# MariusFurter/WeightedSampling.jl

Hardware: AMD Instinct MI355X
Metric: particle-steps/sec (N_particles × T_steps / wall-s), 2D SSM bootstrap filter (higher is better)
Workload: dtype f64; 1 GPU; 2D SSM bootstrap filter (examples/2D_ssm.jl), BASELINE configs[1]; n_particles_per_gpu=1000000, global_particles=1000000, T=100, scheme=stratified, keep_history=True, estimator=reference (single population), parallelism=single GPU

## Files before the change

include/wsmc_math.h:

```cpp
#ifndef WSMC_MATH_H
#define WSMC_MATH_H

#include <stdint.h>

#if defined(__HIPCC__) || defined(__HIP__)
#define WSMC_HD __host__ __device__ inline __attribute__((always_inline))
#else
#define WSMC_HD static inline __attribute__((always_inline))
#endif
#if defined(__clang__)
#define WSMC_UNROLL _Pragma("unroll")
#else
#define WSMC_UNROLL _Pragma("GCC unroll 16")
#endif

typedef unsigned __int128 wsmc_u128;

#if defined(__HIP_DEVICE_COMPILE__)
__device__ inline __attribute__((always_inline)) double wsmc_sreg(double c) {
    __asm__ volatile("" : "+s"(c));
    return c;
}
#define WSMC_K(c) wsmc_sreg(c)
#else
// ... 557 lines not shown
        const double t = y * wsmc_lgamma_g(y);
        return n >= 3.0 ? wsmc_log(z) + t : t;
    }
    const double r = 1.0 / x;
    const double z = r * r;
    double q = WSMC_K(-0.020855820837463117);
    q = __builtin_fma(q, z, WSMC_K(0.0062081367662297935));
    q = __builtin_fma(q, z, WSMC_K(-0.001914965912162907));
    q = __builtin_fma(q, z, WSMC_K(0.0008417325268022405));
    q = __builtin_fma(q, z, WSMC_K(-0.0005952380234291254));
    q = __builtin_fma(q, z, WSMC_K(0.0007936507935117282));
    q = __builtin_fma(q, z, WSMC_K(-0.0027777777777776747));
    q = __builtin_fma(q, z, WSMC_K(0.08333333333333333));
    const double w = __builtin_fma(q, r, 0.4189385332046727);
    const double lx = wsmc_log(x);
    if (lx == WSMC_INF) return lx;
    return __builtin_fma(x - 0.5, lx - 1.0, w);
}
WSMC_HD double wsmc_lgamma3(double a1, double a2, double a3) {
    double acc = 0.0;
#if defined(__clang__)
#pragma nounroll
#endif
    for (int k = 0; k < 3; ++k) {
        const double a = k == 0 ? a1 : (k == 1 ? a2 : a3);
        const double l = a == 1.0 ? 0.0 : wsmc_lgamma(a);
        acc = k == 0 ? l : acc - l;
    }
    return acc;
}
WSMC_HD double wsmc_lbeta(double a, double b) { return -wsmc_lgamma3(a + b, a, b); }
WSMC_HD double wsmc_lchoose(double n, double k) { return wsmc_lgamma3(n + 1.0, k + 1.0, (n - k) + 1.0); }

WSMC_HD void wsmc_normal_pair_t(wsmc_u32x4 w, double* z0, double* z1, const double* logtab) {
    double u1 = wsmc_u01_open0(w.v[0], w.v[1]);
    double u2 = wsmc_u01(w.v[2], w.v[3]);
    double r = wsmc_sqrt(-2.0 * wsmc_log_t(u1, logtab));
    double s, c;
    wsmc_sincos2pi(u2, &s, &c);
    *z0 = r * c; *z1 = r * s;
}
WSMC_HD void wsmc_normal_pair(wsmc_u32x4 w, double* z0, double* z1) { wsmc_normal_pair_t(w, z0, z1, WSMC_LOG_TAB); }
WSMC_HD double wsmc_normal_k(uint64_t seed, uint64_t op, uint64_t idx, uint32_t k) {
    double z0, z1;
    wsmc_normal_pair(wsmc_rng_block(seed, op, idx, k >> 1), &z0, &z1);
    return (k & 1) ? z1 : z0;
}
WSMC_HD double wsmc_uniform_k(uint64_t seed, uint64_t op, uint64_t idx, uint32_t k) {
    wsmc_u32x4 w = wsmc_rng_block(seed, op, idx, (k >> 1) | 0x80u);
    return (k & 1) ? wsmc_u01(w.v[2], w.v[3]) : wsmc_u01(w.v[0], w.v[1]);
}
WSMC_HD uint64_t wsmc_strat_key(uint64_t seed, uint64_t op) {
    uint64_t z = seed ^ (op * 0x9E3779B97F4A7C15ULL) ^ 0x5851F42D4C957F2DULL;
    z ^= z >> 33;
    z *= 0xFF51AFD7ED558CCDULL;
    z ^= z >> 33;
    z *= 0xC4CEB9FE1A85EC53ULL;
    z ^= z >> 33;
    return z;
}
WSMC_HD uint32_t wsmc_strat_fin(uint32_t x) {
    x ^= x >> 16;
    x *= 0x7FEB352Du;
    x ^= x >> 15;
    x *= 0x846CA68Bu;
    x ^= x >> 16;
    return x;
}
WSMC_HD uint32_t wsmc_strat_hash(uint64_t key, uint64_t n) {
    return wsmc_strat_fin((uint32_t)n ^ (uint32_t)key ^ ((uint32_t)(n >> 32) * 0x85EBCA6Bu ^ (uint32_t)(key >> 32)));
}
WSMC_HD uint32_t wsmc_strat_word(uint64_t seed, uint64_t op, uint64_t n) {
    return wsmc_strat_hash(wsmc_strat_key(seed, op), n);
// ... 355 lines not shown
```

weightedsampling.jl_amd/build.py:

```python
from __future__ import annotations

import argparse
import os
import pathlib
import shutil
import subprocess
import sys
from concurrent.futures import ThreadPoolExecutor

PKG = pathlib.Path(__file__).resolve().parent
REPO = PKG.parent
CSRC = PKG / "csrc"
INCLUDE = REPO / "include"
OUT = PKG / "wsmc" / "libwsmc.so"
OBJDIR = PKG / "build"
RESOURCES = OBJDIR / "wsmc_kernels.resources.txt"
SOURCES = ["wsmc_kernels.hip", "wsmc_api.hip", "wsmc_multi.hip", "wsmc_jit.hip", "wsmc_lgssm.hip"]
JIT_HEADERS = [INCLUDE / "wsmc.h", INCLUDE / "wsmc_log_table.h", INCLUDE / "wsmc_exp_table.h", INCLUDE / "wsmc_math.h", INCLUDE / "wsmc_terms.h", CSRC / "wsmc_ew.h",
               CSRC / "wsmc_ew_body.h", CSRC / "wsmc_mv.h", CSRC / "wsmc_mv_body.h"]
ARCH = os.environ.get("WSMC_OFFLOAD_ARCH", "gfx950")


def hipcc() -> str:
    for cand in (os.environ.get("HIPCC"), "/opt/rocm/bin/hipcc", shutil.which("hipcc")):
        if cand and pathlib.Path(cand).exists():
            return cand
    raise RuntimeError("hipcc not found")


COMMON = ["-O3", "-std=c++17", "-fPIC", "-ffp-contract=off", "-fno-fast-math",
          f"--offload-arch={ARCH}", "-I", str(INCLUDE), "-I", str(CSRC),
          "-Wno-unused-result", "-munsafe-fp-atomics"]


def _deps():
    return [CSRC / s for s in SOURCES] + list(CSRC.glob("*.h")) + list(INCLUDE.glob("*.h"))


def up_to_date() -> bool:
    if not OUT.exists() or not RESOURCES.exists():
        return False
    t = OUT.stat().st_mtime
    return all(p.stat().st_mtime <= t for p in _deps())


def write_jit_headers() -> pathlib.Path:
    out = OBJDIR / "wsmc_jit_headers.inc"
    parts = []
    for h in JIT_HEADERS:
        text = h.read_text()
        assert ")WSMCJIT\"" not in text
        parts.append(f'{{"{h.name}", R"WSMCJIT({text})WSMCJIT"}},')
    body = "// generated by build.py: the headers of the run-time compiled kernels\n" + "\n".join(parts) + "\n"
    if not out.exists() or out.read_text() != body:
        out.write_text(body)
    return out


def build(force: bool = False, verbose: bool = False) -> pathlib.Path:
    if not force and up_to_date():
        return OUT
    OBJDIR.mkdir(exist_ok=True)
    write_jit_headers()
    cc = hipcc()

    def compile_one(src: str) -> pathlib.Path:
        obj = OBJDIR / (pathlib.Path(src).stem + ".o")
        cmd = [cc, *COMMON, "-I", str(OBJDIR), "-c", str(CSRC / src), "-o", str(obj)]
        listing = src == "wsmc_kernels.hip"
        if listing:
            cmd.append("-Rpass-analysis=kernel-resource-usage")
        if verbose:
            print(" ".join(cmd), flush=True)
        r = subprocess.run(cmd, capture_output=True, text=True)
        if r.returncode != 0:
            raise RuntimeError(f"hipcc failed on {src}:\n{r.stdout}\n{r.stderr}")
        if listing:
            tail = " [-Rpass-analysis=kernel-resource-usage]"
            remarks = [ln.split("remark: ", 1)[1].replace(tail, "") for ln in r.stderr.splitlines() if "remark: " in ln]
            RESOURCES.write_text("\n".join(remarks) + "\n")
        if verbose and r.stderr and not listing:
            print(r.stderr, file=sys.stderr)
        return obj

    with ThreadPoolExecutor(max_workers=len(SOURCES)) as ex:
        objs = list(ex.map(compile_one, SOURCES))
    tmp = OUT.with_suffix(".so.tmp")
    cmd = [cc, f"--offload-arch={ARCH}", "-shared", "-fPIC", *map(str, objs), "-o", str(tmp),
           "-L/opt/rocm/lib", "-lrccl", "-lhiprtc", "-Wl,-rpath,/opt/rocm/lib"]
    if verbose:
        print(" ".join(cmd), flush=True)
    r = subprocess.run(cmd, capture_output=True, text=True)
    if r.returncode != 0:
        raise RuntimeError(f"link failed:\n{r.stdout}\n{r.stderr}")
    os.replace(tmp, OUT)
    return OUT


if __name__ == "__main__":
    ap = argparse.ArgumentParser()
    ap.add_argument("--force", action="store_true")
    ap.add_argument("--verbose", action="store_true")
    a = ap.parse_args()
    print(build(force=a.force, verbose=a.verbose))
```

weightedsampling.jl_amd/csrc/wsmc_api.hip:

```cpp
#include <hipcub/hipcub.hpp>

#include <algorithm>
#include <chrono>
#include <memory>
#include <thread>
#include <cmath>
#include <cstdio>
#include <cstring>
#include <string>

#include "wsmc_internal.h"

using namespace wsmc;

namespace wsmc {
bool peer_aborted(wsmc_ctx* c) {
    if (!c->peer_abort || !c->peer_abort->load(std::memory_order_acquire)) return false;
    if (c->comm) {
        (void)ncclCommAbort(c->comm);
        c->comm = nullptr;
    }
    c->released = true;
    return true;
}
// ... 555 lines not shown
int wsmc_dist_mvnormal_cov(wsmc_dist* d, const double* cov) {
    if (!d || !cov) return fail(WSMC_EARG, "null argument");
    if (d->dim < 1 || d->dim > WSMC_MVN_MAXDIM) return fail(WSMC_EARG, "MvNormal with a full covariance: dim must be 1..3");
    if (d->mean_fn != WSMC_MEAN_AFFINE) return fail(WSMC_EARG, "MvNormal mean must be affine");
    const int r = wsmc_mvn_pack(d, cov);
    if (r == -1) return fail(WSMC_EARG, "covariance is not symmetric");
    if (r == -2) return fail(WSMC_ENOTPD, "covariance is not positive definite");
    return WSMC_OK;
}

int wsmc_device_count(int32_t* n) {
    int k = 0;
    WSMC_HIP(hipGetDeviceCount(&k));
    *n = k;
    return WSMC_OK;
}

int wsmc_create(wsmc_ctx** out, int64_t n_particles, int32_t device, uint64_t seed) {
    if (!out) return fail(WSMC_EARG, "null out");
    if (n_particles < 1 || n_particles >= (int64_t(1) << 31))
        return fail(WSMC_EARG, "n_particles must be in [1, 2^31)");
    WSMC_HIP(hipSetDevice(device));
    wsmc_ctx* c = new wsmc_ctx();
    c->device = device;
    c->N = n_particles;
    c->gN = n_particles;
    c->seed = seed;
    c->ntiles = (n_particles + kTile - 1) / kTile;
    c->nrstiles = (n_particles + kRsTile - 1) / kRsTile;
    hipError_t e = hipSuccess;
#define ALLOC(ptr, bytes)                                          \
    if (e == hipSuccess) e = hipMalloc((void**)&(ptr), (bytes));
    e = hipStreamCreateWithFlags(&c->stream, hipStreamNonBlocking);
    ALLOC(c->w, sizeof(double) * c->N);
    ALLOC(c->anc, sizeof(int32_t) * c->N);
    ALLOC(c->tmp, sizeof(double) * 4 * c->N);
    ALLOC(c->xchg, sizeof(unsigned long long) * 16 * kMaxWorld);
    ALLOC(c->tilep, sizeof(unsigned long long) * kPart * c->nrstiles);
    ALLOC(c->tileOff, sizeof(unsigned long long) * c->nrstiles);
    ALLOC(c->taskOff, sizeof(int32_t) * c->nrstiles);
    ALLOC(c->taskTile, sizeof(int32_t) * (c->nrstiles + n_particles / kRsChunk + 1));
    ALLOC(c->mslots, sizeof(MaxSlots));
    ALLOC(c->wslots[0], sizeof(MaxSlots));
    ALLOC(c->wslots[1], sizeof(MaxSlots));
    ALLOC(c->qbuf, sizeof(unsigned long long) * c->N);
    ALLOC(c->tilepart, sizeof(double) * 64 * c->ntiles);
    ALLOC(c->rec, sizeof(ShardRecord) * kMaxWorld);
    ALLOC(c->dec, sizeof(Decision));
    ALLOC(c->dec_always, sizeof(Decision));
    ALLOC(c->mom, sizeof(double) * 128);
    ALLOC(c->dflag, sizeof(int32_t) * 4);
    ALLOC(c->ucount, sizeof(unsigned long long) * (4 * kAccMove + 4));
    ALLOC(c->d_colptr, sizeof(double*) * kMaxCols);
    ALLOC(c->run_params, sizeof(uint64_t) * 8);
#undef ALLOC
    if (e == hipSuccess) e = hipHostMalloc(&c->pinned, 4096, hipHostMallocDefault);
    if (e == hipSuccess) e = hipHostMalloc((void**)&c->dec_ring, sizeof(Decision) * kDecRing, hipHostMallocDefault);
    if (e == hipSuccess) e = hipHostGetDevicePointer((void**)&c->dec_ring_dev, c->dec_ring, 0);
    if (e == hipSuccess) e = hipHostGetDevicePointer(&c->pinned_dev, c->pinned, 0);
    if (e == hipSuccess) e = hipMemsetAsync(c->w, 0, sizeof(double) * c->N, c->stream);
    if (e == hipSuccess) e = hipMemsetAsync(c->wslots[0], 0, sizeof(MaxSlots), c->stream);
    if (e == hipSuccess) e = hipMemsetAsync(c->wslots[1], 0, sizeof(MaxSlots), c->stream);
    if (e == hipSuccess) e = hipMemsetAsync(c->anc, 0, sizeof(int32_t) * c->N, c->stream);
    if (e == hipSuccess) {
        Decision always{};
        always.resampled = 1;
        e = hipMemcpy(c->dec_always, &always, sizeof(Decision), hipMemcpyHostToDevice);
    }
    if (e == hipSuccess) e = ctx_sync(c, c->stream);
    {
        const char* eg = getenv("WSMC_EAGER_GATHER");
        c->lazy = !(eg && atoi(eg) != 0);
    }
    if (e != hipSuccess) {
        std::string m = std::string("wsmc_create: ") + hipGetErrorString(e);
        wsmc_destroy(c);
        return fail(WSMC_EHIP, m);
    }
// ... 4203 lines not shown
```

weightedsampling.jl_amd/csrc/wsmc_kernels.hip:

```cpp
#include <hip/hip_ext.h>

#include <cstdlib>
#include "wsmc_internal.h"

namespace wsmc {

typedef double d2 __attribute__((ext_vector_type(2)));

typedef unsigned long long u64;

#ifdef WSMC_DIAG_BUILD
constexpr int kClkKinds = 4, kClkBlocks = 16384;
__device__ u64 g_blk_clk[kClkKinds][kClkBlocks][2];
struct BlkClock {
    int kind;
    u64 t0;
    __device__ __forceinline__ explicit BlkClock(int k) : kind(k), t0(wall_clock64()) {}
    __device__ __forceinline__ ~BlkClock() {
        if (threadIdx.x == 0 && blockIdx.x < (unsigned)kClkBlocks) {
            g_blk_clk[kind][blockIdx.x][0] = t0;
            g_blk_clk[kind][blockIdx.x][1] = wall_clock64();
        }
    }
};
// ... 20 lines not shown
}
__device__ __forceinline__ u64 lane63_u64(u64 v) {
    const uint32_t lo = (uint32_t)__builtin_amdgcn_readlane((int)(uint32_t)v, 63);
    const uint32_t hi = (uint32_t)__builtin_amdgcn_readlane((int)(uint32_t)(v >> 32), 63);
    return ((u64)hi << 32) | lo;
}
__device__ __forceinline__ u64 wave_sum_u64(u64 v) {
    v += dpp_u64<kDppQuad1032>(v);
    v += dpp_u64<kDppQuad2301>(v);
    v += dpp_u64<kDppRowRor4>(v);
    v += dpp_u64<kDppRowRor8>(v);
    v += dpp_u64<kDppBcast15>(v);
    v += dpp_u64<kDppBcast31>(v);
    return lane63_u64(v);
}
__device__ __forceinline__ u64 wave_max_u64(u64 v) {
    u64 o;
    o = dpp_u64<kDppQuad1032>(v); v = o > v ? o : v;
    o = dpp_u64<kDppQuad2301>(v); v = o > v ? o : v;
    o = dpp_u64<kDppRowRor4>(v); v = o > v ? o : v;
    o = dpp_u64<kDppRowRor8>(v); v = o > v ? o : v;
    o = dpp_u64<kDppBcast15>(v); v = o > v ? o : v;
    o = dpp_u64<kDppBcast31>(v); v = o > v ? o : v;
    return lane63_u64(v);
}
__device__ __forceinline__ double wave_sum_f64_exact(double v) {
    v = v + dpp_f64<kDppQuad1032>(v);
    v = v + dpp_f64<kDppQuad2301>(v);
    v = v + dpp_f64<kDppRowRor4>(v);
    v = v + dpp_f64<kDppRowRor8>(v);
    v = v + dpp_f64<kDppBcast15>(v);
    v = v + dpp_f64<kDppBcast31>(v);
    return __builtin_bit_cast(double, lane63_u64(__builtin_bit_cast(u64, v)));
}
__device__ __forceinline__ u64 wave_incl_scan_u64(u64 v) {
    u64 x = v + dpp_u64<kDppRowShr1>(v);
    x += dpp_u64<kDppRowShr2>(v);
    x += dpp_u64<kDppRowShr3>(v);
    x += dpp_u64<kDppRowShr4, 0xf, 0xe>(x);
    x += dpp_u64<kDppRowShr8, 0xf, 0xc>(x);
    x += dpp_u64<kDppBcast15, 0xa, 0xf>(x);
    x += dpp_u64<kDppBcast31, 0xc, 0xf>(x);
    return x;
}
__device__ __forceinline__ double block_sum_canon(double v, double* lds4) {
#pragma unroll
    for (int off = 1; off < 64; off <<= 1) v = v + __shfl_xor(v, off, 64);
    if ((threadIdx.x & 63) == 0) lds4[threadIdx.x >> 6] = v;
    __syncthreads();
    double r = (lds4[0] + lds4[1]) + (lds4[2] + lds4[3]);
    __syncthreads();
    return r;
}
__device__ __forceinline__ u64 block_sum_u64(u64 v, u64* lds4) {
    v = wave_sum_u64(v);
    if ((threadIdx.x & 63) == 0) lds4[threadIdx.x >> 6] = v;
    __syncthreads();
    u64 r = (lds4[0] + lds4[1]) + (lds4[2] + lds4[3]);
    __syncthreads();
    return r;
}
__device__ __forceinline__ u64 block_max_u64(u64 v, u64* lds4) {
    v = wave_max_u64(v);
    if ((threadIdx.x & 63) == 0) lds4[threadIdx.x >> 6] = v;
    __syncthreads();
    u64 a = lds4[0] > lds4[1] ? lds4[0] : lds4[1];
// ... 879 lines not shown
            if (dd < -kMargin) return ns;
        }
    }
    return wsmc_rank_r(c, Q, N, ratio, scheme, seed, op, slot_base);
}

template <int CTRL, int ROW = 0xf, int BANK = 0xf>
__device__ __forceinline__ int dpp_i32_or(int v, int idn) {
    return __builtin_amdgcn_update_dpp(idn, v, CTRL, ROW, BANK, false);
}
__device__ __forceinline__ int wave_incl_max_i32(int v) {
    int x = max(v, dpp_i32_or<kDppRowShr1>(v, -1));
    x = max(x, dpp_i32_or<kDppRowShr2>(v, -1));
    x = max(x, dpp_i32_or<kDppRowShr3>(v, -1));
    x = max(x, dpp_i32_or<kDppRowShr4, 0xf, 0xe>(x, -1));
    x = max(x, dpp_i32_or<kDppRowShr8, 0xf, 0xc>(x, -1));
    x = max(x, dpp_i32_or<kDppBcast15, 0xa, 0xf>(x, -1));
    x = max(x, dpp_i32_or<kDppBcast31, 0xc, 0xf>(x, -1));
    return x;
}
__device__ __forceinline__ double wave_incl_scan_f64(double v) {
    double x = v + dpp_f64<kDppRowShr1>(v);
    x = x + dpp_f64<kDppRowShr2>(v);
    x = x + dpp_f64<kDppRowShr3>(v);
    x = x + __builtin_bit_cast(double, dpp_u64<kDppRowShr4, 0xf, 0xe>(__builtin_bit_cast(u64, x)));
    x = x + __builtin_bit_cast(double, dpp_u64<kDppRowShr8, 0xf, 0xc>(__builtin_bit_cast(u64, x)));
    x = x + __builtin_bit_cast(double, dpp_u64<kDppBcast15, 0xa, 0xf>(__builtin_bit_cast(u64, x)));
    x = x + __builtin_bit_cast(double, dpp_u64<kDppBcast31, 0xc, 0xf>(__builtin_bit_cast(u64, x)));
    return x;
}

template <int IT>
__device__ __forceinline__ void load_tile_q(int64_t N, int b, const u64* __restrict__ qbuf, u64 (&q)[IT]) {
#pragma unroll
    for (int k = 0; k < IT; ++k) {
        const int64_t i = (int64_t)b * kRsTile + (int64_t)threadIdx.x * IT + k;
        q[k] = i < N ? qbuf[i] : 0ull;
    }
}

template <int IT>
__device__ __forceinline__ void load_tile_qw(int64_t N, int b, const double* __restrict__ w,
                                             const MaxSlots* __restrict__ ms, const double* rref, u64 (&q)[IT]) {
    double lw[IT];
#pragma unroll
    for (int k = 0; k < IT; ++k) {
        const int64_t i = (int64_t)b * kRsTile + (int64_t)threadIdx.x * IT + k;
        lw[k] = i < N ? w[i] : -WSMC_INF;
    }
    const double R = rref ? *rref : wsmc_qref(wave_slots_max(ms));
    const double sK = wsmc_pow2i(wsmc_qbits((uint64_t)N));
#pragma unroll
    for (int k = 0; k < IT; ++k) {
        double e = wsmc_expw(lw[k] - R);
        e = e > 0.0 ? e : 0.0;
        q[k] = d_small_to_u64(wsmc_floor(e * sK));
    }
}

__device__ __forceinline__ void fill_clear(FillLds& sh) {
    const int4 m1 = make_int4(-1, -1, -1, -1);
    int4* o = reinterpret_cast<int4*>(sh.out);
    o[2 * threadIdx.x] = m1;
    o[2 * threadIdx.x + 1] = m1;
    if (threadIdx.x == 0) o[2 * kScanBlock] = m1;
}

__device__ __forceinline__ void fill_store4(int32_t* __restrict__ dst, int p0, int a, int e, int4 v) {
    if (p0 >= a && p0 + 4 <= e) {
        *reinterpret_cast<int4*>(dst + p0) = v;
    } else if (p0 + 4 > a && p0 < e) {
        if (p0 >= a && p0 < e) dst[p0] = v.x;
        if (p0 + 1 >= a && p0 + 1 < e) dst[p0 + 1] = v.y;
        if (p0 + 2 >= a && p0 + 2 < e) dst[p0 + 2] = v.z;
        if (p0 + 3 >= a && p0 + 3 < e) dst[p0 + 3] = v.w;
    }
}

template <int MODE>
__device__ __forceinline__ void fill_chunk_core(int64_t N, int b, int j, u64 Q, u64 off, u64 qb, double pre,
                                                const FillPlan& plan, uint64_t opx,
                                                const u64 (&q)[kRsTile / kScanBlock], int32_t* __restrict__ anc,
// ... 583 lines not shown
        if ((th & 63) == 0)
#pragma unroll
            for (int k = 0; k < kRedPart; ++k) s_parts[th >> 6][k] = acc[k];
        __syncthreads();
        if (th == 0) {
            u64 tot[kRedPart] = {0, 0, 0, 0, 0, 0};
            for (int v = 0; v < kScanBlock / 64; ++v)
                for (int k = 0; k < kRedPart; ++k) tot[k] += s_parts[v][k];
            ShardRecord r;
            r.menc = menc;
            r.Q = tot[0];
            r.q2 = tot[1];
            const wsmc_u128 Wf2 = (wsmc_u128)tot[2] + ((wsmc_u128)tot[3] << 32);
            const wsmc_u128 Wf = (wsmc_u128)tot[4] + ((wsmc_u128)tot[5] << 32);
            r.wf2lo = (u64)Wf2; r.wf2hi = (u64)(Wf2 >> 64);
            r.wflo = (u64)Wf; r.wfhi = (u64)(Wf >> 64);
            r.n = (u64)N;
            *rec = r;
            if (plan.rg_check && !(wsmc_qref(wsmc_ord_dec(menc)) == *plan.rg_check)) atomicAdd(plan.rg_miss, 1);
            if (dec) {
                decide_records(&r, 1, 0, ess_min, dec);
                if (plan.host_dec) *plan.host_dec = *dec;
                if (plan.base_out) *plan.base_out = dec->resampled ? dec->mean : wsmc_ord_dec(menc);
                if (plan.ms_reset && dec->resampled) {
                    plan.ms_reset->v[0][0] = wsmc_ord_enc(dec->mean);
                    for (int k = 1; k < kSlots; ++k) plan.ms_reset->v[k][0] = 0ull;
                }
            }
        }
        return;
    }
    const uint64_t opx = op_eff(plan.op, plan.op_dev);
    if (t < ntiles) {
        u64 q[kRsTile / kScanBlock];
        if (QW)
            load_tile_qw(N, t, wq, ms, plan.rg_check, q);
        else
            load_tile_q(N, t, qbuf, q);
        const u64 qb = plan.tilep[(int64_t)t * kPart];
        const int g = t / G;
        u64 pre = 0, tot = 0;
        if (plan.xlines) {
            const int ngw = (int)(plan.xstride / kGroupLine);
            for (int k = th; k < plan.dx_world * ngw; k += kScanBlock) {
                const int r = k / ngw, kk = k - r * ngw;
                const u64 v = plan.xlines[(int64_t)r * plan.xstride + (int64_t)kk * kGroupLine];
                tot += v;
                pre += (r < plan.dx_rank || (r == plan.dx_rank && kk < g)) ? v : 0ull;
            }
        } else {
            for (int k = th; k < ngroups; k += kScanBlock) {
                const u64 v = grp[(int64_t)k * 8];
                tot += v;
                pre += k < g ? v : 0ull;
            }
        }
        for (int b = g * G + th; b < t; b += kScanBlock) pre += plan.tilep[(int64_t)b * kPart];
        fill_clear(sh);
        const int lane = th & 63, wv = th >> 6;
        pre = wave_sum_u64(pre);
        tot = wave_sum_u64(tot);
        const double tsum = tile_q_sum(q);
        const double x = wave_incl_scan_f64(tsum);
        if (lane == 63) {
            sh.uw[wv] = x;
            sh.red[wv][0] = pre;
            sh.red[wv][1] = tot;
        }
        __syncthreads();
        u64 off = 0, Q = 0;
        double lp = 0.0;
#pragma unroll
        for (int k = 0; k < kScanBlock / 64; ++k) {
            off += sh.red[k][0];
            Q += sh.red[k][1];
            if (k < wv) lp = lp + sh.uw[k];
        }
        fill_chunk_core<0>(N, t, 0, Q, off, qb, lp + (x - tsum), plan, opx, q, anc, sh, false);
        return;
    }
    u64 Q = 0, qmax = 0, cbase = 0;
    for (int k = th; k < ngroups; k += kScanBlock) {
        Q += grp[(int64_t)k * kGroupLine];
        const u64 m = grp[(int64_t)k * kGroupLine + 1];
        qmax = m > qmax ? m : qmax;
    }
    if (plan.xlines) {
        Q = 0;
        const int ngw = (int)(plan.xstride / kGroupLine);
        for (int k = th; k < plan.dx_world * ngw; k += kScanBlock) {
            const int r = k / ngw, kk = k - r * ngw;
            const u64 v = plan.xlines[(int64_t)r * plan.xstride + (int64_t)kk * kGroupLine];
            Q += v;
            cbase += r < plan.dx_rank ? v : 0ull;
        }
    }
    qmax = block_max_u64(qmax, s_u);
    block_sum2_u64(Q, cbase, s_red);
    const uint64_t Nr = plan.n_global ? plan.n_global : (uint64_t)N;
    const double ratio = Q ? wsmc_u64_to_d(Nr) / wsmc_u64_to_d(Q) : 0.0;
    if (ovf_chunks(qmax, ratio) == 0) return;

    const int per = (ntiles + kScanBlock - 1) / kScanBlock;
    const int b0 = th * per < ntiles ? th * per : ntiles;
    const int b1 = b0 + per < ntiles ? b0 + per : ntiles;
    u64 qs = 0, ns = 0;
    for (int b = b0; b < b1; ++b) {
        const u64 qb = plan.tilep[(int64_t)b * kPart];
        qs += qb;
        ns += (u64)ovf_chunks(qb, ratio);
    }
    u64 qtot, ntasks;
    const u64 qpre = block_excl_scan_u64<kScanBlock / 64>(qs, s_u, &qtot);
    const u64 npre = block_excl_scan_u64<kScanBlock / 64>(ns, s_u, &ntasks);
    __shared__ uint32_t s_npre[kScanBlock], s_ns[kScanBlock];
    __shared__ u64 s_c0[kScanBlock];
    s_npre[th] = (uint32_t)npre;
    s_ns[th] = (uint32_t)ns;
    s_c0[th] = cbase + qpre;
    const u64 Qu = ((u64)__builtin_amdgcn_readfirstlane((int)(Q >> 32)) << 32) |
                   (uint32_t)__builtin_amdgcn_readfirstlane((int)(uint32_t)Q);
    const uint32_t nt = (uint32_t)__builtin_amdgcn_readfirstlane((int)(uint32_t)ntasks);
    for (uint32_t o = (uint32_t)(t - ntiles); o < nt; o += kOverflowBlocks) {
        const uint32_t n0_ = s_npre[th], k_ = s_ns[th];
        if (o >= n0_ && o < n0_ + k_) {
            u64 c = s_c0[th];
            uint32_t n0 = n0_;
            const int per_ = (ntiles + kScanBlock - 1) / kScanBlock;
            const int bb0 = th * per_ < ntiles ? th * per_ : ntiles;
            const int bb1 = bb0 + per_ < ntiles ? bb0 + per_ : ntiles;
            for (int b = bb0; b < bb1; ++b) {
                const u64 qb = plan.tilep[(int64_t)b * kPart];
                const uint32_t k = (uint32_t)ovf_chunks(qb, ratio);
                if (o < n0 + k) {
// ... 1037 lines not shown
    const bool isl = QS ? ISL : (a.recs_prev != nullptr && a.t > 1);
    const bool identity = !QS && a.identity;
    const int64_t stride = (int64_t)gridDim.x * NT * 2;
    const int64_t ib = ((int64_t)blockIdx.x * NT + threadIdx.x) * 2;
    int2 s2[IT];
    bool ok[IT], two[IT];
#pragma unroll
    for (int j = 0; j < IT; ++j) {
        const int64_t i0 = ib + (int64_t)j * stride;
        ok[j] = i0 < N;
        two[j] = i0 + 1 < N;
        s2[j] = int2{0, 0};
        if (QS && (MODE & 2) == 0) {
            s2[j] = *reinterpret_cast<const int2*>(a.anc_prev + (ok[j] ? i0 : 0));
        } else if (ok[j] && !first && (MODE & 2) == 0 && !identity) {
            if (two[j]) {
                s2[j] = *reinterpret_cast<const int2*>(a.anc_prev + i0);
            } else {
                s2[j].x = a.anc_prev[i0];
            }
        }
    }
    u64 mprev = 0;
    if (QS) mprev = a.ms_prev->v[threadIdx.x & 63][0];
    if (isl) {
        if (threadIdx.x == 0) {
            Decision dd;
            decide_records(a.recs_prev, a.world, a.rank, a.ess_min, &dd);
            s_dec = dd;
            if (blockIdx.x == 0) *a.dec_out = dd;
        }
    }
    const uint64_t op_dv = a.op_dev[0] + 3ull * (uint64_t)(a.t - 1);
    const double o0 = a.obs[2 * (a.t - 1)], o1 = a.obs[2 * (a.t - 1) + 1];
    bool rs = false;
    double mean = 0.0;
    if (!isl && !first) {
        rs = a.dec_prev->resampled;
        mean = rs ? a.dec_prev->mean : 0.0;
    }
    if (WSMC_PROP_LDS_LOG && (MODE & 1) == 0) {
        const double* lt = wsmc_log_table();
        for (int k = (int)threadIdx.x; k < 2 * WSMC_LOG_TABLE_N; k += NT) s_logtab[k] = lt[k];
    }
    if ((WSMC_PROP_LDS_LOG && (MODE & 1) == 0) || isl) __syncthreads();
    const double* logtab = WSMC_PROP_LDS_LOG ? s_logtab : wsmc_log_table();
    if (isl) {
        rs = s_dec.resampled;
        mean = rs ? s_dec.mean : 0.0;
    }
    int64_t src[IT][2];
#pragma unroll
    for (int j = 0; j < IT; ++j) {
        const int64_t i0 = ib + (int64_t)j * stride;
        src[j][0] = i0; src[j][1] = i0 + 1;
        if (ok[j] && !first && (MODE & 2) == 0 && !identity && rs) { src[j][0] = s2[j].x; src[j][1] = s2[j].y; }
    }
    d2 xp[IT][2], vp[IT][2];
    double wb[IT][2];
#pragma unroll
    for (int j = 0; j < IT; ++j) {
        const int64_t i0 = ib + (int64_t)j * stride;
        wb[j][0] = wb[j][1] = mean;
        if (!ok[j]) continue;
        if (!rs) {
            if (two[j]) {
                const d2 w2 = *reinterpret_cast<const d2*>(a.w + i0);
                wb[j][0] = w2.x; wb[j][1] = w2.y;
                if (!QS && a.w_save) *reinterpret_cast<d2*>(a.w_save + i0) = w2;
            } else {
                wb[j][0] = a.w[i0];
                if (!QS && a.w_save) a.w_save[i0] = wb[j][0];
            }
        }
#pragma unroll
        for (int k = 0; k < 2; ++k) {
            if (first) {
                xp[j][k] = d2{a.x0[0], a.x0[1]};
                vp[j][k] = d2{a.v0[0], a.v0[1]};
            } else if (k == 0 || two[j]) {
                if (MODE & 16) {
                    const int64_t loc = rs ? src[j][k] - a.goff : src[j][k];
                    const bool here = loc >= 0 && loc < N;
                    const double* xs = here ? a.x_prev + 2 * loc : a.xr + 2 * (i0 + k);
                    const double* vs = here ? a.v_prev + 2 * loc : a.vr + 2 * (i0 + k);
                    xp[j][k] = *reinterpret_cast<const d2*>(xs);
                    vp[j][k] = *reinterpret_cast<const d2*>(vs);
                } else {
                    xp[j][k] = *reinterpret_cast<const d2*>(a.x_prev + 2 * src[j][k]);
                    vp[j][k] = *reinterpret_cast<const d2*>(a.v_prev + 2 * src[j][k]);
                }
            }
        }
    }
    u64 menc = 0;
    QAcc acc;
    double Rg = 0.0, sK = 0.0;
    if (QS) {
        const double base = rs ? mean : wsmc_ord_dec(wave_max_u64(mprev));
        const double lpmax = -(a.c0 + 0.0) * 0.5;
        Rg = wsmc_qref(base + lpmax);
        sK = wsmc_pow2i(wsmc_qbits((uint64_t)N));
        if (blockIdx.x == 0 && threadIdx.x == 0) *a.rg_out = Rg;
    }
#pragma unroll
    for (int j = 0; j < IT; ++j) {
        if (!ok[j]) continue;
        const int64_t i0 = ib + (int64_t)j * stride;
        double z[2][2] = {{0.0, 0.0}, {0.0, 0.0}};
        if ((MODE & 1) == 0) {
#pragma unroll
            for (int k = 0; k < 2; ++k)
                wsmc_normal_pair_t(wsmc_rng_block(a.seed, op_dv, (uint64_t)(a.goff + i0 + k), 0u), &z[k][0], &z[k][1],
                                   logtab);
        }
        d2 xn[2], vn[2], dvv[2];
        double wn[2];
#pragma unroll
        for (int k = 0; k < 2; ++k) {
            const double xn0 = aff2(xp[j][k].x, vp[j][k].x), xn1 = aff2(xp[j][k].y, vp[j][k].y);
            const double dv0 = 0.0 + a.q_sd * z[k][0], dv1 = 0.0 + a.q_sd * z[k][1];
            const double vn0 = aff2(vp[j][k].x, dv0), vn1 = aff2(vp[j][k].y, dv1);
            const double m0 = 0.0 + 1.0 * xn0, m1 = 0.0 + 1.0 * xn1;
            double s = 0.0;
            const double d0 = o0 - m0, d1 = o1 - m1;
            s = s + d0 * d0;
            s = s + d1 * d1;
            const double lp = -(a.c0 + s / a.r_var) * 0.5;
            wn[k] = wb[j][k] + lp;
            xn[k] = d2{xn0, xn1};
            vn[k] = d2{vn0, vn1};
            dvv[k] = d2{dv0, dv1};
        }
        *reinterpret_cast<d2*>(a.x_next + 2 * i0) = xn[0];
        *reinterpret_cast<d2*>(a.v_next + 2 * i0) = vn[0];
        if (a.dv) *reinterpret_cast<d2*>(a.dv + 2 * i0) = dvv[0];
        u64 e0 = wsmc_ord_enc(wn[0]);
        menc = e0 > menc ? e0 : menc;
        u64 q0 = 0, q1 = 0;
        if (QS) q0 = qacc_add(acc, wsmc_expw(wn[0] - Rg), sK);
        if (two[j]) {
            *reinterpret_cast<d2*>(a.x_next + 2 * i0 + 2) = xn[1];
            *reinterpret_cast<d2*>(a.v_next + 2 * i0 + 2) = vn[1];
            if (a.dv) *reinterpret_cast<d2*>(a.dv + 2 * i0 + 2) = dvv[1];
            *reinterpret_cast<d2*>(a.w + i0) = d2{wn[0], wn[1]};
            const u64 e1 = wsmc_ord_enc(wn[1]);
            menc = e1 > menc ? e1 : menc;
            if (QS) q1 = qacc_add(acc, wsmc_expw(wn[1] - Rg), sK);
            if (QS && a.qbuf) *reinterpret_cast<ulonglong2*>(a.qbuf + i0) = make_ulonglong2(q0, q1);
        } else {
            a.w[i0] = wn[0];
            if (QS && a.qbuf) a.qbuf[i0] = q0;
        }
    }
    if (QS) {
        __shared__ double s_f[kPart][NT / 64];
        const int th = threadIdx.x, wv = th >> 6;
        acc.Q = wave_sum_f64_exact(acc.Q);
        acc.Q2 = wave_sum_f64_exact(acc.Q2);
        acc.WF2 = wave_sum_f64_exact(acc.WF2);
        acc.WF = wave_sum_f64_exact(acc.WF);
        menc = wave_max_u64(menc);
        if ((th & 63) == 0) {
            s_f[0][wv] = acc.Q; s_f[1][wv] = acc.Q2;
            s_f[2][wv] = acc.WF2; s_f[3][wv] = acc.WF;
            lds4[wv] = menc;
        }
        __syncthreads();
        if (th < kPart) {
            double f = 0.0;
#pragma unroll
            for (int v = 0; v < NT / 64; ++v) f = f + s_f[th][v];
            const u64 t = (u64)f;
            a.tilep[(int64_t)blockIdx.x * kPart + th] = t;
            if (th == 0) {
                u64* gl = a.grp + (int64_t)(blockIdx.x / a.G) * kGroupLine;
                atomicAdd(gl, t);
                atomicMax(gl + 1, t);
            }
        } else if (th == 64) {
            u64 m = 0;
#pragma unroll
            for (int v = 0; v < NT / 64; ++v) m = lds4[v] > m ? lds4[v] : m;
            atomic_max_filtered(&a.ms->v[blockIdx.x % kSlots][0], m);
        }
        return;
    }
    if (MODE & 4) {
        if (menc == 0x123456789ull) a.w[0] = 0.0;
        return;
    }
    if (MODE & 8) {
        menc = wave_max_u64(menc);
        if ((threadIdx.x & 63) == 0) atomicMax(&a.ms->v[(blockIdx.x * 4 + (threadIdx.x >> 6)) % kSlots][0], menc);
        return;
    }
    menc = block_max_u64(menc, lds4);
    if (threadIdx.x == 0) atomic_max_filtered(&a.ms->v[blockIdx.x % kSlots][0], menc);
}

__global__ __launch_bounds__(kBlock) void k_trace_pack(const double* __restrict__ xpairs,
                                                       const int32_t* __restrict__ arow, int64_t start, int64_t count,
                                                       u64* __restrict__ out) {
    const int64_t j = (int64_t)blockIdx.x * kBlock + threadIdx.x;
    if (j >= count) return;
    const d2 x = *reinterpret_cast<const d2*>(xpairs + 2 * (start + j));
    out[3 * j] = (u64)wsmc_d2bits(x.x);
    out[3 * j + 1] = (u64)wsmc_d2bits(x.y);
    out[3 * j + 2] = arow ? (u64)(uint32_t)arow[start + j] : 0ull;
}
__global__ __launch_bounds__(kBlock) void k_trace_lookup(const u64* __restrict__ recv, int64_t lo,
                                                         const int32_t* __restrict__ a, int64_t n,
                                                         double* __restrict__ xout, int32_t* __restrict__ anext,
                                                         int use_a) {
    const int64_t i = (int64_t)blockIdx.x * kBlock + threadIdx.x;
    if (i >= n) return;
    const int64_t o = (int64_t)a[i] - lo;
    xout[i] = wsmc_bits2d(recv[3 * o]);
    xout[n + i] = wsmc_bits2d(recv[3 * o + 1]);
    anext[i] = use_a ? (int32_t)(uint32_t)recv[3 * o + 2] : a[i];
}
__global__ __launch_bounds__(kBlock) void k_pairs_to_soa(const double* __restrict__ pairs, double* __restrict__ soa,
                                                         int64_t n) {
    const int64_t i = (int64_t)blockIdx.x * kBlock + threadIdx.x;
    if (i >= n) return;
    const d2 v = *reinterpret_cast<const d2*>(pairs + 2 * i);
    soa[i] = v.x;
    soa[n + i] = v.y;
}
__global__ __launch_bounds__(kBlock) void k_fill_const2(double* __restrict__ soa, double v0, double v1, int64_t n) {
    const int64_t i = (int64_t)blockIdx.x * kBlock + threadIdx.x;
    if (i >= n) return;
// ... 1057 lines not shown
```

Baseline: 32.57 billion particle-steps/s.

## Split normal draws around log-table staging and vectorize tile/quad reductions

In the fused 2D SSM propagate kernel, the Box-Muller draw is split into a head (uniforms and sincos), computed before the LDS log-table barrier, and a tail (log and sqrt), so the RNG work overlaps the table staging. Kernel arguments are re-read late through an opaque kernarg pointer to lower scalar register pressure. The per-wave four-value reduction is merged into one permlane-swap tree. Loads in the resample scan are vectorized to quads, and its prefix loads are hoisted, which needs the weight and qbuf buffers padded to a multiple of four. The build also emits an ISA listing.

```diff
diff --git a/include/wsmc_math.h b/include/wsmc_math.h
--- a/include/wsmc_math.h
+++ b/include/wsmc_math.h
@@ -613,13 +613,18 @@
 WSMC_HD double wsmc_lbeta(double a, double b) { return -wsmc_lgamma3(a + b, a, b); }
 WSMC_HD double wsmc_lchoose(double n, double k) { return wsmc_lgamma3(n + 1.0, k + 1.0, (n - k) + 1.0); }
 
+WSMC_HD void wsmc_normal_pair_head(wsmc_u32x4 w, double* u1, double* s, double* c) {
+    *u1 = wsmc_u01_open0(w.v[0], w.v[1]);
+    wsmc_sincos2pi(wsmc_u01(w.v[2], w.v[3]), s, c);
+}
+WSMC_HD void wsmc_normal_pair_tail(double u1, double s, double c, double* z0, double* z1, const double* logtab) {
+    double r = wsmc_sqrt(-2.0 * wsmc_log_t(u1, logtab));
+    *z0 = r * c; *z1 = r * s;
+}
 WSMC_HD void wsmc_normal_pair_t(wsmc_u32x4 w, double* z0, double* z1, const double* logtab) {
-    double u1 = wsmc_u01_open0(w.v[0], w.v[1]);
-    double u2 = wsmc_u01(w.v[2], w.v[3]);
-    double r = wsmc_sqrt(-2.0 * wsmc_log_t(u1, logtab));
-    double s, c;
-    wsmc_sincos2pi(u2, &s, &c);
-    *z0 = r * c; *z1 = r * s;
+    double u1, s, c;
+    wsmc_normal_pair_head(w, &u1, &s, &c);
+    wsmc_normal_pair_tail(u1, s, c, z0, z1, logtab);
 }
 WSMC_HD void wsmc_normal_pair(wsmc_u32x4 w, double* z0, double* z1) { wsmc_normal_pair_t(w, z0, z1, WSMC_LOG_TAB); }
 WSMC_HD double wsmc_normal_k(uint64_t seed, uint64_t op, uint64_t idx, uint32_t k) {
diff --git a/weightedsampling.jl_amd/build.py b/weightedsampling.jl_amd/build.py
--- a/weightedsampling.jl_amd/build.py
+++ b/weightedsampling.jl_amd/build.py
@@ -15,6 +15,7 @@
 OUT = PKG / "wsmc" / "libwsmc.so"
 OBJDIR = PKG / "build"
 RESOURCES = OBJDIR / "wsmc_kernels.resources.txt"
+ISA = OBJDIR / "wsmc_kernels.s"
 SOURCES = ["wsmc_kernels.hip", "wsmc_api.hip", "wsmc_multi.hip", "wsmc_jit.hip", "wsmc_lgssm.hip"]
 JIT_HEADERS = [INCLUDE / "wsmc.h", INCLUDE / "wsmc_log_table.h", INCLUDE / "wsmc_exp_table.h", INCLUDE / "wsmc_math.h", INCLUDE / "wsmc_terms.h", CSRC / "wsmc_ew.h",
                CSRC / "wsmc_ew_body.h", CSRC / "wsmc_mv.h", CSRC / "wsmc_mv_body.h"]
@@ -38,7 +39,7 @@
 
 
 def up_to_date() -> bool:
-    if not OUT.exists() or not RESOURCES.exists():
+    if not OUT.exists() or not RESOURCES.exists() or not ISA.exists():
         return False
     t = OUT.stat().st_mtime
     return all(p.stat().st_mtime <= t for p in _deps())
@@ -83,8 +84,20 @@
             print(r.stderr, file=sys.stderr)
         return obj
 
-    with ThreadPoolExecutor(max_workers=len(SOURCES)) as ex:
+    def listing_isa() -> None:
+        tmp = ISA.with_suffix(".s.tmp")
+        cmd = [cc, *COMMON, "-I", str(OBJDIR), "--offload-device-only", "-S", str(CSRC / "wsmc_kernels.hip"), "-o", str(tmp)]
+        if verbose:
+            print(" ".join(cmd), flush=True)
+        r = subprocess.run(cmd, capture_output=True, text=True)
+        if r.returncode != 0:
+            raise RuntimeError(f"hipcc -S failed on wsmc_kernels.hip:\n{r.stdout}\n{r.stderr}")
+        os.replace(tmp, ISA)
+
+    with ThreadPoolExecutor(max_workers=len(SOURCES) + 1) as ex:
+        isa = ex.submit(listing_isa)
         objs = list(ex.map(compile_one, SOURCES))
+        isa.result()
     tmp = OUT.with_suffix(".so.tmp")
     cmd = [cc, f"--offload-arch={ARCH}", "-shared", "-fPIC", *map(str, objs), "-o", str(tmp),
            "-L/opt/rocm/lib", "-lrccl", "-lhiprtc", "-Wl,-rpath,/opt/rocm/lib"]
diff --git a/weightedsampling.jl_amd/csrc/wsmc_api.hip b/weightedsampling.jl_amd/csrc/wsmc_api.hip
--- a/weightedsampling.jl_amd/csrc/wsmc_api.hip
+++ b/weightedsampling.jl_amd/csrc/wsmc_api.hip
@@ -611,7 +611,7 @@
 #define ALLOC(ptr, bytes)                                          \
     if (e == hipSuccess) e = hipMalloc((void**)&(ptr), (bytes));
     e = hipStreamCreateWithFlags(&c->stream, hipStreamNonBlocking);
-    ALLOC(c->w, sizeof(double) * c->N);
+    ALLOC(c->w, sizeof(double) * ((c->N + 3) & ~(int64_t)3));
     ALLOC(c->anc, sizeof(int32_t) * c->N);
     ALLOC(c->tmp, sizeof(double) * 4 * c->N);
     ALLOC(c->xchg, sizeof(unsigned long long) * 16 * kMaxWorld);
@@ -622,7 +622,7 @@
     ALLOC(c->mslots, sizeof(MaxSlots));
     ALLOC(c->wslots[0], sizeof(MaxSlots));
     ALLOC(c->wslots[1], sizeof(MaxSlots));
-    ALLOC(c->qbuf, sizeof(unsigned long long) * c->N);
+    ALLOC(c->qbuf, sizeof(unsigned long long) * ((c->N + 3) & ~(int64_t)3));
     ALLOC(c->tilepart, sizeof(double) * 64 * c->ntiles);
     ALLOC(c->rec, sizeof(ShardRecord) * kMaxWorld);
     ALLOC(c->dec, sizeof(Decision));
diff --git a/weightedsampling.jl_amd/csrc/wsmc_kernels.hip b/weightedsampling.jl_amd/csrc/wsmc_kernels.hip
--- a/weightedsampling.jl_amd/csrc/wsmc_kernels.hip
+++ b/weightedsampling.jl_amd/csrc/wsmc_kernels.hip
@@ -76,6 +76,32 @@
     v = v + dpp_f64<kDppBcast15>(v);
     v = v + dpp_f64<kDppBcast31>(v);
     return __builtin_bit_cast(double, lane63_u64(__builtin_bit_cast(u64, v)));
+}
+__device__ __forceinline__ void lane_swap32(double& a, double& b) {
+    const u64 x = __builtin_bit_cast(u64, a), y = __builtin_bit_cast(u64, b);
+    const auto lo = __builtin_amdgcn_permlane32_swap((uint32_t)x, (uint32_t)y, false, false);
+    const auto hi = __builtin_amdgcn_permlane32_swap((uint32_t)(x >> 32), (uint32_t)(y >> 32), false, false);
+    a = __builtin_bit_cast(double, ((u64)hi[0] << 32) | lo[0]);
+    b = __builtin_bit_cast(double, ((u64)hi[1] << 32) | lo[1]);
+}
+__device__ __forceinline__ void lane_swap16(double& a, double& b) {
+    const u64 x = __builtin_bit_cast(u64, a), y = __builtin_bit_cast(u64, b);
+    const auto lo = __builtin_amdgcn_permlane16_swap((uint32_t)x, (uint32_t)y, false, false);
+    const auto hi = __builtin_amdgcn_permlane16_swap((uint32_t)(x >> 32), (uint32_t)(y >> 32), false, false);
+    a = __builtin_bit_cast(double, ((u64)hi[0] << 32) | lo[0]);
+    b = __builtin_bit_cast(double, ((u64)hi[1] << 32) | lo[1]);
+}
+__device__ __forceinline__ double wave_sum4_f64_exact(double v0, double v1, double v2, double v3) {
+    lane_swap32(v0, v2);
+    lane_swap32(v1, v3);
+    double a = v0 + v2, b = v1 + v3;
+    lane_swap16(a, b);
+    double r = a + b;
+    r = r + dpp_f64<kDppQuad1032>(r);
+    r = r + dpp_f64<kDppQuad2301>(r);
+    r = r + dpp_f64<kDppRowRor4>(r);
+    r = r + dpp_f64<kDppRowRor8>(r);
+    return r;
 }
 __device__ __forceinline__ u64 wave_incl_scan_u64(u64 v) {
     u64 x = v + dpp_u64<kDppRowShr1>(v);
@@ -1021,22 +1047,28 @@
 
 template <int IT>
 __device__ __forceinline__ void load_tile_q(int64_t N, int b, const u64* __restrict__ qbuf, u64 (&q)[IT]) {
-#pragma unroll
-    for (int k = 0; k < IT; ++k) {
-        const int64_t i = (int64_t)b * kRsTile + (int64_t)threadIdx.x * IT + k;
-        q[k] = i < N ? qbuf[i] : 0ull;
-    }
+    static_assert(IT == 4, "one quad a thread");
+    const int64_t i = (int64_t)b * kRsTile + (int64_t)threadIdx.x * IT;
+    const ulonglong2* p = reinterpret_cast<const ulonglong2*>(qbuf + (i < N ? i : 0));
+    const ulonglong2 lo = p[0], hi = p[1];
+    q[0] = i < N ? lo.x : 0ull;
+    q[1] = i + 1 < N ? lo.y : 0ull;
+    q[2] = i + 2 < N ? hi.x : 0ull;
+    q[3] = i + 3 < N ? hi.y : 0ull;
 }
 
 template <int IT>
 __device__ __forceinline__ void load_tile_qw(int64_t N, int b, const double* __restrict__ w,
                                              const MaxSlots* __restrict__ ms, const double* rref, u64 (&q)[IT]) {
+    static_assert(IT == 4, "one quad a thread");
+    const int64_t i = (int64_t)b * kRsTile + (int64_t)threadIdx.x * IT;
+    const d2* p = reinterpret_cast<const d2*>(w + (i < N ? i : 0));
+    const d2 lo = p[0], hi = p[1];
     double lw[IT];
-#pragma unroll
-    for (int k = 0; k < IT; ++k) {
-        const int64_t i = (int64_t)b * kRsTile + (int64_t)threadIdx.x * IT + k;
-        lw[k] = i < N ? w[i] : -WSMC_INF;
-    }
+    lw[0] = i < N ? lo.x : -WSMC_INF;
+    lw[1] = i + 1 < N ? lo.y : -WSMC_INF;
+    lw[2] = i + 2 < N ? hi.x : -WSMC_INF;
+    lw[3] = i + 3 < N ? hi.y : -WSMC_INF;
     const double R = rref ? *rref : wsmc_qref(wave_slots_max(ms));
     const double sK = wsmc_pow2i(wsmc_qbits((uint64_t)N));
 #pragma unroll
@@ -1686,13 +1718,16 @@
     }
     const uint64_t opx = op_eff(plan.op, plan.op_dev);
     if (t < ntiles) {
+        const u64 qb = plan.tilep[(int64_t)t * kPart];
+        const int g = t / G;
+        const u64 g0 = grp[(int64_t)(th < ngroups ? th : 0) * 8];
+        const int bf = g * G + th;
+        const u64 p0 = plan.tilep[(int64_t)(bf < t ? bf : t) * kPart];
         u64 q[kRsTile / kScanBlock];
         if (QW)
             load_tile_qw(N, t, wq, ms, plan.rg_check, q);
         else
             load_tile_q(N, t, qbuf, q);
-        const u64 qb = plan.tilep[(int64_t)t * kPart];
-        const int g = t / G;
         u64 pre = 0, tot = 0;
         if (plan.xlines) {
             const int ngw = (int)(plan.xstride / kGroupLine);
@@ -1703,13 +1738,16 @@
                 pre += (r < plan.dx_rank || (r == plan.dx_rank && kk < g)) ? v : 0ull;
             }
         } else {
-            for (int k = th; k < ngroups; k += kScanBlock) {
+            tot = th < ngroups ? g0 : 0ull;
+            pre = th < g ? g0 : 0ull;
+            for (int k = th + kScanBlock; k < ngroups; k += kScanBlock) {
                 const u64 v = grp[(int64_t)k * 8];
                 tot += v;
                 pre += k < g ? v : 0ull;
             }
         }
-        for (int b = g * G + th; b < t; b += kScanBlock) pre += plan.tilep[(int64_t)b * kPart];
+        pre += bf < t ? p0 : 0ull;
+        for (int b = bf + kScanBlock; b < t; b += kScanBlock) pre += plan.tilep[(int64_t)b * kPart];
         fill_clear(sh);
         const int lane = th & 63, wv = th >> 6;
         pre = wave_sum_u64(pre);
@@ -1752,8 +1790,10 @@
     qmax = block_max_u64(qmax, s_u);
     block_sum2_u64(Q, cbase, s_red);
     const uint64_t Nr = plan.n_global ? plan.n_global : (uint64_t)N;
-    const double ratio = Q ? wsmc_u64_to_d(Nr) / wsmc_u64_to_d(Q) : 0.0;
-    if (ovf_chunks(qmax, ratio) == 0) return;
+    const double ratio_v = Q ? wsmc_u64_to_d(Nr) / wsmc_u64_to_d(Q) : 0.0;
+    if (ovf_chunks(qmax, ratio_v) == 0) return;
+    const double ratio = __builtin_bit_cast(double, ((u64)__builtin_amdgcn_readfirstlane((int)(__builtin_bit_cast(u64, ratio_v) >> 32)) << 32) |
+                                                        (uint32_t)__builtin_amdgcn_readfirstlane((int)(uint32_t)__builtin_bit_cast(u64, ratio_v)));
 
     const int per = (ntiles + kScanBlock - 1) / kScanBlock;
     const int b0 = th * per < ntiles ? th * per : ntiles;
@@ -2857,19 +2897,38 @@
         }
     }
     const uint64_t op_dv = a.op_dev[0] + 3ull * (uint64_t)(a.t - 1);
-    const double o0 = a.obs[2 * (a.t - 1)], o1 = a.obs[2 * (a.t - 1) + 1];
     bool rs = false;
     double mean = 0.0;
     if (!isl && !first) {
         rs = a.dec_prev->resampled;
         mean = rs ? a.dec_prev->mean : 0.0;
     }
-    if (WSMC_PROP_LDS_LOG && (MODE & 1) == 0) {
+    constexpr bool kSplitDraw = QS && IT == 1 && WSMC_PROP_LDS_LOG && (MODE & 1) == 0 && 2 * WSMC_LOG_TABLE_N <= NT;
+    double du1[2] = {0.0, 0.0}, dsn[2] = {0.0, 0.0}, dcs[2] = {0.0, 0.0};
+    uint32_t koff = 0;
+    if (kSplitDraw) {
+        const double tv = wsmc_log_table()[threadIdx.x & (2 * WSMC_LOG_TABLE_N - 1)];
+        __builtin_amdgcn_sched_barrier(0);
+#pragma unroll
+        for (int k = 0; k < 2; ++k)
+            wsmc_normal_pair_head(wsmc_rng_block(a.seed, op_dv, (uint64_t)(a.goff + ib + k), 0u), &du1[k], &dsn[k], &dcs[k]);
+#pragma unroll
+        for (int k = 0; k < 2; ++k) asm volatile("" : "+v"(du1[k]), "+v"(dsn[k]), "+v"(dcs[k]));
+        asm volatile("" : "+s"(koff));
+        __builtin_amdgcn_sched_barrier(0);
+        s_logtab[threadIdx.x & (2 * WSMC_LOG_TABLE_N - 1)] = tv;
+    } else if (WSMC_PROP_LDS_LOG && (MODE & 1) == 0) {
         const double* lt = wsmc_log_table();
         for (int k = (int)threadIdx.x; k < 2 * WSMC_LOG_TABLE_N; k += NT) s_logtab[k] = lt[k];
     }
     if ((WSMC_PROP_LDS_LOG && (MODE & 1) == 0) || isl) __syncthreads();
     const double* logtab = WSMC_PROP_LDS_LOG ? s_logtab : wsmc_log_table();
+    typedef const char __attribute__((address_space(4)))* KargBytes;
+    typedef const Ssm2dArgs __attribute__((address_space(4)))* KargP;
+    const KargP ka = (KargP)((KargBytes)__builtin_amdgcn_kernarg_segment_ptr() + koff);
+#define ARG_LATE(f) (kSplitDraw ? ka->f : a.f)
+    const double* const obs_t = ARG_LATE(obs) + 2 * (a.t - 1);
+    const double o0 = obs_t[0], o1 = obs_t[1];
     if (isl) {
         rs = s_dec.resampled;
         mean = rs ? s_dec.mean : 0.0;
@@ -2887,14 +2946,27 @@
     for (int j = 0; j < IT; ++j) {
         const int64_t i0 = ib + (int64_t)j * stride;
         wb[j][0] = wb[j][1] = mean;
+        if (QS) {
+            if (!rs) {
+                const d2 w2 = *reinterpret_cast<const d2*>(ARG_LATE(w) + (ok[j] ? i0 : 0));
+                wb[j][0] = w2.x; wb[j][1] = w2.y;
+            }
+#pragma unroll
+            for (int k = 0; k < 2; ++k) {
+                const int64_t sk = (k == 0 ? ok[j] : two[j]) ? src[j][k] : 0;
+                xp[j][k] = *reinterpret_cast<const d2*>(ARG_LATE(x_prev) + 2 * sk);
+                vp[j][k] = *reinterpret_cast<const d2*>(ARG_LATE(v_prev) + 2 * sk);
+            }
+            continue;
+        }
         if (!ok[j]) continue;
         if (!rs) {
             if (two[j]) {
-                const d2 w2 = *reinterpret_cast<const d2*>(a.w + i0);
+                const d2 w2 = *reinterpret_cast<const d2*>(ARG_LATE(w) + i0);
                 wb[j][0] = w2.x; wb[j][1] = w2.y;
                 if (!QS && a.w_save) *reinterpret_cast<d2*>(a.w_save + i0) = w2;
             } else {
-                wb[j][0] = a.w[i0];
+                wb[j][0] = ARG_LATE(w)[i0];
                 if (!QS && a.w_save) a.w_save[i0] = wb[j][0];
             }
         }
@@ -2907,13 +2979,13 @@
                 if (MODE & 16) {
                     const int64_t loc = rs ? src[j][k] - a.goff : src[j][k];
                     const bool here = loc >= 0 && loc < N;
-                    const double* xs = here ? a.x_prev + 2 * loc : a.xr + 2 * (i0 + k);
-                    const double* vs = here ? a.v_prev + 2 * loc : a.vr + 2 * (i0 + k);
+                    const double* xs = here ? ARG_LATE(x_prev) + 2 * loc : a.xr + 2 * (i0 + k);
+                    const double* vs = here ? ARG_LATE(v_prev) + 2 * loc : a.vr + 2 * (i0 + k);
                     xp[j][k] = *reinterpret_cast<const d2*>(xs);
                     vp[j][k] = *reinterpret_cast<const d2*>(vs);
                 } else {
-                    xp[j][k] = *reinterpret_cast<const d2*>(a.x_prev + 2 * src[j][k]);
-                    vp[j][k] = *reinterpret_cast<const d2*>(a.v_prev + 2 * src[j][k]);
+                    xp[j][k] = *reinterpret_cast<const d2*>(ARG_LATE(x_prev) + 2 * src[j][k]);
+                    vp[j][k] = *reinterpret_cast<const d2*>(ARG_LATE(v_prev) + 2 * src[j][k]);
                 }
             }
         }
@@ -2923,17 +2995,26 @@
     double Rg = 0.0, sK = 0.0;
     if (QS) {
         const double base = rs ? mean : wsmc_ord_dec(wave_max_u64(mprev));
-        const double lpmax = -(a.c0 + 0.0) * 0.5;
+        const double lpmax = -(ARG_LATE(c0) + 0.0) * 0.5;
         Rg = wsmc_qref(base + lpmax);
         sK = wsmc_pow2i(wsmc_qbits((uint64_t)N));
-        if (blockIdx.x == 0 && threadIdx.x == 0) *a.rg_out = Rg;
+        if (blockIdx.x == 0 && threadIdx.x == 0) *ARG_LATE(rg_out) = Rg;
+    }
+    double zs[2][2] = {{0.0, 0.0}, {0.0, 0.0}};
+    if (kSplitDraw) {
+        __builtin_amdgcn_sched_barrier(0);
+#pragma unroll
+        for (int k = 0; k < 2; ++k) wsmc_normal_pair_tail(du1[k], dsn[k], dcs[k], &zs[k][0], &zs[k][1], logtab);
+#pragma unroll
+        for (int k = 0; k < 2; ++k) asm volatile("" : "+v"(zs[k][0]), "+v"(zs[k][1]));
+        __builtin_amdgcn_sched_barrier(0);
     }
 #pragma unroll
     for (int j = 0; j < IT; ++j) {
         if (!ok[j]) continue;
         const int64_t i0 = ib + (int64_t)j * stride;
-        double z[2][2] = {{0.0, 0.0}, {0.0, 0.0}};
-        if ((MODE & 1) == 0) {
+        double z[2][2] = {{zs[0][0], zs[0][1]}, {zs[1][0], zs[1][1]}};
+        if (!kSplitDraw && (MODE & 1) == 0) {
 #pragma unroll
             for (int k = 0; k < 2; ++k)
                 wsmc_normal_pair_t(wsmc_rng_block(a.seed, op_dv, (uint64_t)(a.goff + i0 + k), 0u), &z[k][0], &z[k][1],
@@ -2944,62 +3025,56 @@
 #pragma unroll
         for (int k = 0; k < 2; ++k) {
             const double xn0 = aff2(xp[j][k].x, vp[j][k].x), xn1 = aff2(xp[j][k].y, vp[j][k].y);
-            const double dv0 = 0.0 + a.q_sd * z[k][0], dv1 = 0.0 + a.q_sd * z[k][1];
+            const double dv0 = 0.0 + ARG_LATE(q_sd) * z[k][0], dv1 = 0.0 + ARG_LATE(q_sd) * z[k][1];
             const double vn0 = aff2(vp[j][k].x, dv0), vn1 = aff2(vp[j][k].y, dv1);
             const double m0 = 0.0 + 1.0 * xn0, m1 = 0.0 + 1.0 * xn1;
             double s = 0.0;
             const double d0 = o0 - m0, d1 = o1 - m1;
             s = s + d0 * d0;
             s = s + d1 * d1;
-            const double lp = -(a.c0 + s / a.r_var) * 0.5;
+            const double lp = -(ARG_LATE(c0) + s / ARG_LATE(r_var)) * 0.5;
             wn[k] = wb[j][k] + lp;
             xn[k] = d2{xn0, xn1};
             vn[k] = d2{vn0, vn1};
             dvv[k] = d2{dv0, dv1};
         }
-        *reinterpret_cast<d2*>(a.x_next + 2 * i0) = xn[0];
-        *reinterpret_cast<d2*>(a.v_next + 2 * i0) = vn[0];
-        if (a.dv) *reinterpret_cast<d2*>(a.dv + 2 * i0) = dvv[0];
+        *reinterpret_cast<d2*>(ARG_LATE(x_next) + 2 * i0) = xn[0];
+        *reinterpret_cast<d2*>(ARG_LATE(v_next) + 2 * i0) = vn[0];
+        if (ARG_LATE(dv)) *reinterpret_cast<d2*>(ARG_LATE(dv) + 2 * i0) = dvv[0];
         u64 e0 = wsmc_ord_enc(wn[0]);
         menc = e0 > menc ? e0 : menc;
         u64 q0 = 0, q1 = 0;
         if (QS) q0 = qacc_add(acc, wsmc_expw(wn[0] - Rg), sK);
         if (two[j]) {
-            *reinterpret_cast<d2*>(a.x_next + 2 * i0 + 2) = xn[1];
-            *reinterpret_cast<d2*>(a.v_next + 2 * i0 + 2) = vn[1];
-            if (a.dv) *reinterpret_cast<d2*>(a.dv + 2 * i0 + 2) = dvv[1];
-            *reinterpret_cast<d2*>(a.w + i0) = d2{wn[0], wn[1]};
+            *reinterpret_cast<d2*>(ARG_LATE(x_next) + 2 * i0 + 2) = xn[1];
+            *reinterpret_cast<d2*>(ARG_LATE(v_next) + 2 * i0 + 2) = vn[1];
+            if (ARG_LATE(dv)) *reinterpret_cast<d2*>(ARG_LATE(dv) + 2 * i0 + 2) = dvv[1];
+            *reinterpret_cast<d2*>(ARG_LATE(w) + i0) = d2{wn[0], wn[1]};
             const u64 e1 = wsmc_ord_enc(wn[1]);
             menc = e1 > menc ? e1 : menc;
             if (QS) q1 = qacc_add(acc, wsmc_expw(wn[1] - Rg), sK);
-            if (QS && a.qbuf) *reinterpret_cast<ulonglong2*>(a.qbuf + i0) = make_ulonglong2(q0, q1);
+            if (QS && ARG_LATE(qbuf)) *reinterpret_cast<ulonglong2*>(ARG_LATE(qbuf) + i0) = make_ulonglong2(q0, q1);
         } else {
-            a.w[i0] = wn[0];
-            if (QS && a.qbuf) a.qbuf[i0] = q0;
+            ARG_LATE(w)[i0] = wn[0];
+            if (QS && ARG_LATE(qbuf)) ARG_LATE(qbuf)[i0] = q0;
         }
     }
     if (QS) {
         __shared__ double s_f[kPart][NT / 64];
         const int th = threadIdx.x, wv = th >> 6;
-        acc.Q = wave_sum_f64_exact(acc.Q);
-        acc.Q2 = wave_sum_f64_exact(acc.Q2);
-        acc.WF2 = wave_sum_f64_exact(acc.WF2);
-        acc.WF = wave_sum_f64_exact(acc.WF);
+        const double part = wave_sum4_f64_exact(acc.Q, acc.Q2, acc.WF2, acc.WF);
         menc = wave_max_u64(menc);
-        if ((th & 63) == 0) {
-            s_f[0][wv] = acc.Q; s_f[1][wv] = acc.Q2;
-            s_f[2][wv] = acc.WF2; s_f[3][wv] = acc.WF;
-            lds4[wv] = menc;
-        }
+        if ((th & 15) == 0) s_f[(th & 63) >> 4][wv] = part;
+        if ((th & 63) == 0) lds4[wv] = menc;
         __syncthreads();
         if (th < kPart) {
             double f = 0.0;
 #pragma unroll
             for (int v = 0; v < NT / 64; ++v) f = f + s_f[th][v];
             const u64 t = (u64)f;
-            a.tilep[(int64_t)blockIdx.x * kPart + th] = t;
+            ARG_LATE(tilep)[(int64_t)blockIdx.x * kPart + th] = t;
             if (th == 0) {
-                u64* gl = a.grp + (int64_t)(blockIdx.x / a.G) * kGroupLine;
+                u64* gl = ARG_LATE(grp) + (int64_t)(blockIdx.x / ARG_LATE(G)) * kGroupLine;
                 atomicAdd(gl, t);
                 atomicMax(gl + 1, t);
             }
@@ -3007,22 +3082,23 @@
             u64 m = 0;
 #pragma unroll
             for (int v = 0; v < NT / 64; ++v) m = lds4[v] > m ? lds4[v] : m;
-            atomic_max_filtered(&a.ms->v[blockIdx.x % kSlots][0], m);
+            atomic_max_filtered(&ARG_LATE(ms)->v[blockIdx.x % kSlots][0], m);
         }
         return;
     }
     if (MODE & 4) {
-        if (menc == 0x123456789ull) a.w[0] = 0.0;
+        if (menc == 0x123456789ull) ARG_LATE(w)[0] = 0.0;
         return;
     }
     if (MODE & 8) {
         menc = wave_max_u64(menc);
-        if ((threadIdx.x & 63) == 0) atomicMax(&a.ms->v[(blockIdx.x * 4 + (threadIdx.x >> 6)) % kSlots][0], menc);
+        if ((threadIdx.x & 63) == 0) atomicMax(&ARG_LATE(ms)->v[(blockIdx.x * 4 + (threadIdx.x >> 6)) % kSlots][0], menc);
         return;
     }
     menc = block_max_u64(menc, lds4);
-    if (threadIdx.x == 0) atomic_max_filtered(&a.ms->v[blockIdx.x % kSlots][0], menc);
-}
+    if (threadIdx.x == 0) atomic_max_filtered(&ARG_LATE(ms)->v[blockIdx.x % kSlots][0], menc);
+}
+#undef ARG_LATE
 
 __global__ __launch_bounds__(kBlock) void k_trace_pack(const double* __restrict__ xpairs,
                                                        const int32_t* __restrict__ arow, int64_t start, int64_t count,
```

Result: faster. 33.93 billion particle-steps/s (median of 6 runs) (+4.2%).
